# nnaisense/evotorch

Hardware: NVIDIA H100
Metric: PGPE generations/sec at popsize=1Mxdim=10k (Rastrigin, fp32) (higher is better)
Workload: dtype f32

## Files before the change

evotorch_b200/csrc/evok_common.cuh:

```cuda
#pragma once

#include <cuda_runtime.h>
#include <stdint.h>

#include "../../include/evok.h"
#include "evok_sampler.cuh"

#define EVOK_CHECK_LAUNCH_N(n)                       \
  do {                                               \
    cudaError_t e__ = cudaPeekAtLastError();         \
    if (e__ != cudaSuccess) return (int)e__;         \
    evok::count_launches(n);                         \
  } while (0)
#define EVOK_CHECK_LAUNCH() EVOK_CHECK_LAUNCH_N(1)

namespace evok {

extern unsigned long long g_launch_count;
inline void count_launches(int n) { __atomic_fetch_add(&g_launch_count, (unsigned long long)n, __ATOMIC_RELAXED); }

constexpr int kWarp = 32;
constexpr int kNumSMs = 132;
constexpr int64_t kMaxGridY = 65535;

template <typename Fn>
inline int for_item_chunks(int64_t n_items, int64_t max_items, Fn&& fn) {
  for (int64_t b0 = 0; b0 < n_items; b0 += max_items) {
    const int rc = fn(b0, n_items - b0 < max_items ? n_items - b0 : max_items);
    if (rc) return rc;
  }
  return 0;
}

inline PhiloxKey make_philox_key(uint64_t seed, uint64_t stream_id) {
  PhiloxKey k;
  uint32_t a = (uint32_t)seed, b = (uint32_t)(seed >> 32) ^ (uint32_t)(stream_id >> 32);
  for (int r = 0; r < 10; ++r) {
    k.k0[r] = a;
    k.k1[r] = b;
    a += 0x9E3779B9u;
    b += 0xBB67AE85u;
  }
  k.stream_lo = (uint32_t)stream_id;
  return k;
}

template <typename T>
__device__ __forceinline__ T block_sum(T v, T* smem ) {
  const int lane = threadIdx.x & 31, wid = threadIdx.x >> 5, nw = (blockDim.x + 31) >> 5;
  v = warp_sum(v);
  __syncthreads();
  if (lane == 0) smem[wid] = v;
  __syncthreads();
  if (wid == 0) {
    T t = lane < nw ? smem[lane] : T(0);
    t = warp_sum(t);
    if (lane == 0) smem[32] = t;
  }
  __syncthreads();
  return smem[32];
}

inline bool aligned16(const void* p) { return (reinterpret_cast<uintptr_t>(p) & 15u) == 0; }
__device__ __forceinline__ bool aligned16_dev(const void* p) { return (reinterpret_cast<uintptr_t>(p) & 15u) == 0; }

__device__ __forceinline__ float tanh_1e6(float x) {
  const float ax = fabsf(x);
  float r;
  if (ax < 0.25f) {
    const float t = ax * ax;
    r = ax * fmaf(t, fmaf(t, fmaf(t, fmaf(t, 0.021869488f, -0.053968254f), 0.13333334f), -0.33333334f), 1.0f);
  } else {
    const float e = __expf(-2.0f * ax);
    r = __fdividef(1.0f - e, 1.0f + e);
  }
  return copysignf(r, x);
}
__device__ __forceinline__ float tanh_abs1e7(float x) {
  const float e = __expf(-2.0f * fabsf(x));
  return copysignf(__fdividef(1.0f - e, 1.0f + e), x);
}
__device__ __forceinline__ float activate_fast(float v, int act) {
  switch (act) {
    case EVOK_ACT_TANH: return tanh_1e6(v);
    case EVOK_ACT_RELU: return fmaxf(v, 0.0f);
    case EVOK_ACT_SIGMOID: return __fdividef(1.0f, 1.0f + __expf(-v));
    default: return v;
  }
}

}
```

evotorch_b200/csrc/evok_grad.cu:

```cuda
#include <dlfcn.h>

#include <atomic>
#include <cstdlib>

#include "evok_common.cuh"

#ifndef EVOK_GRAD_TMA_DEFAULT
#define EVOK_GRAD_TMA_DEFAULT 1
#endif

namespace evok {

constexpr int kGradThreads = 256;
constexpr int kGradUnroll = 4;
constexpr int kGradMinBlocks = 4;
constexpr int kGradCtasPerSm = 4;
constexpr int kMaxResidentCtas = kNumSMs * 8;

template <int VEC>
struct VecF;
template <>
struct VecF<4> {
  float v[4];
};
// ... 160 lines not shown
        }
      }
    }
  }

  __shared__ float red[TY > 1 ? TY : 1][TX][2 * VEC];
  if (TY > 1) {
#pragma unroll
    for (int c = 0; c < VEC; ++c) {
      red[ty][tx][c] = s1[c];
      red[ty][tx][VEC + c] = s2[c];
    }
    __syncthreads();
    if (ty == 0) {
#pragma unroll
      for (int c = 0; c < VEC; ++c) {
        float t1 = red[0][tx][c], t2 = red[0][tx][VEC + c];
        for (int y = 1; y < TY; ++y) {
          t1 += red[y][tx][c];
          t2 += red[y][tx][VEC + c];
        }
        s1[c] = t1;
        s2[c] = t2;
      }
    }
  }
  if (ty == 0 && active) store_partial<VEC>(partial, blockIdx.y, D, col, s1, s2);
  if (SEPW && blockIdx.x == 0) {
    __shared__ float wred[TY];
    if (tx == 0) wred[ty] = wb;
    __syncthreads();
    if (threadIdx.x == 0) {
      float t = wred[0];
      for (int y = 1; y < TY; ++y) t += wred[y];
      wsum_partial[blockIdx.y] = t;
    }
  }
}

__device__ __forceinline__ void sum_chunks(const float* __restrict__ partial, int n_chunks, int64_t D, int64_t j, float& t1, float& t2) {
  t1 = 0.0f;
  t2 = 0.0f;
  for (int c = 0; c < n_chunks; ++c) {
    t1 += partial[((int64_t)c * 2 + 0) * D + j];
    t2 += partial[((int64_t)c * 2 + 1) * D + j];
  }
}

template <bool WSUM = false>
__global__ void __launch_bounds__(256) grad_finalize_kernel(const float* __restrict__ partial, int n_chunks, int64_t D, float scale_mu,
                                                            float scale_sigma, float* __restrict__ out_mu, float* __restrict__ out_sigma,
                                                            int64_t item_stride_partial = 0, const float* __restrict__ wsum_partial = nullptr,
                                                            float* __restrict__ wsum_out = nullptr) {
  const int64_t j = (int64_t)blockIdx.x * blockDim.x + threadIdx.x;
  if (WSUM && j == 0) {
    wsum_partial += (int64_t)blockIdx.y * n_chunks;
    float t = 0.0f;
    for (int c = 0; c < n_chunks; ++c) t += wsum_partial[c];
    wsum_out[blockIdx.y] = t;
  }
  if (j >= D) return;
  partial += (int64_t)blockIdx.y * item_stride_partial;
  out_mu += (int64_t)blockIdx.y * D;
  out_sigma += (int64_t)blockIdx.y * D;
  float t1, t2;
  sum_chunks(partial, n_chunks, D, j, t1, t2);
  out_mu[j] = t1 * scale_mu;
  out_sigma[j] = t2 * scale_sigma;
}

template <int EPS>
__global__ void __launch_bounds__(256) sepcma_sqnorm_kernel(const float* __restrict__ X, int64_t item_stride_x, int64_t ldx, const float* __restrict__ m,
                                                            const float* __restrict__ s, const float* __restrict__ aw, int64_t n_rows, int64_t D,
                                                            const __grid_constant__ PhiloxKey key, float* __restrict__ q) {
  const int lane = threadIdx.x & 31;
  const int64_t row = (int64_t)blockIdx.x * 8 + (threadIdx.x >> 5);
  if (row >= n_rows) return;
  const int64_t item = blockIdx.y;
  aw += item * n_rows;
  q += item * n_rows;
  if (!(__ldg(aw + row) < 0.0f)) return;
  m += item * D;
  s += item * D;
  const float* x_row = EPS == kEpsRead ? X + item * item_stride_x + row * ldx : nullptr;
  const bool vec = EPS == kEpsRead && (D & 3) == 0 && aligned16_dev(x_row);
  const uint32_t sw = key.stream_lo + (uint32_t)item;
  float acc = 0.0f;
  for (int64_t g = lane; 4 * g < D; g += 32) {
    const int64_t col = 4 * g;
    float x[4];
    if (EPS == kEpsRebuild) {
      float z[4];
      normals4(key, sw, (uint64_t)row, (uint32_t)g, z);
#pragma unroll
      for (int c = 0; c < 4; ++c) x[c] = col + c < D ? fmaf(__ldg(s + col + c), z[c], __ldg(m + col + c)) : 0.0f;
    } else if (vec) {
      const float4 v = ld_stream4(x_row + col);
      x[0] = v.x; x[1] = v.y; x[2] = v.z; x[3] = v.w;
    } else {
#pragma unroll
      for (int c = 0; c < 4; ++c) x[c] = col + c < D ? ld_stream1(x_row + col + c) : 0.0f;
    }
#pragma unroll
    for (int c = 0; c < 4; ++c) {
      if (col + c < D) {
        const float z = __fdiv_rn(x[c] - __ldg(m + col + c), __ldg(s + col + c));
        acc = fmaf(z, z, acc);
      }
    }
  }
  acc = warp_sum(acc);
  if (lane == 0) q[row] = acc;
}

struct GradPush {
  PeerSink sink;
  const unsigned long long* epoch;
  unsigned int* done;
};

__global__ void __launch_bounds__(256) grad_finalize_push_kernel(const float* __restrict__ partial, int n_chunks, int64_t D, float scale_mu,
                                                                 float scale_sigma, const __grid_constant__ PeerSink sink,
                                                                 const unsigned long long* epoch, unsigned int* done) {
  const int64_t j = (int64_t)blockIdx.x * blockDim.x + threadIdx.x;
  if (j < D) {
    float t1, t2;
    sum_chunks(partial, n_chunks, D, j, t1, t2);
    t1 *= scale_mu;
    t2 *= scale_sigma;
    for (int p = 0; p < sink.world; ++p) {
      float* slot = static_cast<float*>(sink.data[p]) + (int64_t)sink.rank * 2 * D;
      slot[j] = t1;
      slot[D + j] = t2;
    }
  }
  peer_signal_tail(sink, epoch, done);
}

#ifndef EVOK_GRAD_TMA_ROWS
#define EVOK_GRAD_TMA_ROWS 4
#endif
#ifndef EVOK_GRAD_TMA_STAGES
#define EVOK_GRAD_TMA_STAGES 4
#endif
#ifndef EVOK_GRAD_TMA_CTAS_PER_SM
#define EVOK_GRAD_TMA_CTAS_PER_SM 3
#endif
constexpr int kTmaRows = EVOK_GRAD_TMA_ROWS;
constexpr int kTmaStages = EVOK_GRAD_TMA_STAGES;
constexpr int kTmaCols = 1024;
constexpr int kTmaConsumers = 256;
constexpr int kTmaThreads = kTmaConsumers + 32;
constexpr size_t kTmaSmemBytes = (size_t)kTmaStages * kTmaRows * kTmaCols * sizeof(float) + 2 * kTmaStages * sizeof(uint64_t) + 128;

__device__ __forceinline__ uint32_t smem_u32(const void* p) { return (uint32_t)__cvta_generic_to_shared(p); }
__device__ __forceinline__ void mbar_init(uint64_t* bar, uint32_t count) {
  asm volatile("mbarrier.init.shared::cta.b64 [%0], %1;" ::"r"(smem_u32(bar)), "r"(count) : "memory");
}
__device__ __forceinline__ void mbar_expect_tx(uint64_t* bar, uint32_t bytes) {
  asm volatile("mbarrier.arrive.expect_tx.shared::cta.b64 _, [%0], %1;" ::"r"(smem_u32(bar)), "r"(bytes) : "memory");
}
__device__ __forceinline__ void mbar_arrive(uint64_t* bar) {
  asm volatile("mbarrier.arrive.shared::cta.b64 _, [%0];" ::"r"(smem_u32(bar)) : "memory");
}
__device__ __forceinline__ void mbar_wait(uint64_t* bar, uint32_t parity) {
  asm volatile(
      "{\n"
      ".reg .pred P1;\n"
      "LAB_WAIT:\n"
      "mbarrier.try_wait.parity.shared::cta.b64 P1, [%0], %1;\n"
      "@P1 bra DONE;\n"
      "bra LAB_WAIT;\n"
      "DONE:\n"
      "}" ::"r"(smem_u32(bar)), "r"(parity) : "memory");
}
__device__ __forceinline__ void bulk_load(void* dst_smem, const void* src_gmem, uint32_t bytes, uint64_t* bar) {
  asm volatile("cp.async.bulk.shared::cluster.global.mbarrier::complete_tx::bytes [%0], [%1], %2, [%3];" ::"r"(smem_u32(dst_smem)),
               "l"(src_gmem), "r"(bytes), "r"(smem_u32(bar))
               : "memory");
}

constexpr int kSplitPeriod = 16;
__device__ __forceinline__ uint32_t rebuilt_mask(int split) {
  uint32_t m = 0;
#pragma unroll
  for (int k = 0; k < kSplitPeriod; ++k)
    if ((k + 1) * split / kSplitPeriod > k * split / kSplitPeriod) m |= 1u << k;
  return m;
}
__device__ __forceinline__ bool group_rebuilt(uint32_t mask, int64_t g) { return (mask >> ((int)g & (kSplitPeriod - 1))) & 1u; }

template <bool SYM>
__global__ void __launch_bounds__(kTmaThreads, EVOK_GRAD_TMA_CTAS_PER_SM)
    grad_partial_tma_kernel(int form, const float* __restrict__ X, int64_t ldx, const float* __restrict__ w, const float* __restrict__ mu,
                            const float* __restrict__ sigma, int64_t n_units, int64_t D, int64_t units_per_chunk, int split, uint64_t unit0,
                            const __grid_constant__ PhiloxKey key, const uint32_t* __restrict__ stream_off, float* __restrict__ partial) {
  extern __shared__ __align__(128) unsigned char smem_raw[];
  float* tiles = reinterpret_cast<float*>(smem_raw);
  uint64_t* full = reinterpret_cast<uint64_t*>(smem_raw + (size_t)kTmaStages * kTmaRows * kTmaCols * sizeof(float));
  uint64_t* empty = full + kTmaStages;

  const int tid = threadIdx.x, warp = tid >> 5, lane = tid & 31;
  const int64_t col0 = (int64_t)blockIdx.x * kTmaCols;
  const int64_t width = min((int64_t)kTmaCols, D - col0);
  const int64_t r_begin = (int64_t)blockIdx.y * units_per_chunk;
  const int64_t r_end = min(n_units, r_begin + units_per_chunk);
  const int64_t n_rows = r_end - r_begin;
  const int64_t n_groups = (n_rows + kTmaRows - 1) / kTmaRows;
  const int64_t row_stride = (SYM ? 2 : 1) * ldx;
  const uint32_t mask = rebuilt_mask(split);

  if (tid == 0) {
    for (int s = 0; s < kTmaStages; ++s) {
      mbar_init(&full[s], 1);
      mbar_init(&empty[s], kTmaConsumers / 32);
    }
    asm volatile("fence.mbarrier_init.release.cluster;" ::: "memory");
  }
  __syncthreads();

  if (warp == kTmaConsumers / 32) {
    if (lane == 0) {
      const uint32_t row_bytes = (uint32_t)(width * sizeof(float));
      int64_t t = 0;
      for (int64_t g = 0; g < n_groups; ++g) {
        if (group_rebuilt(mask, g)) continue;
        const int s = (int)(t % kTmaStages);
        const uint32_t use = (uint32_t)(t / kTmaStages);
        ++t;
        if (use > 0) mbar_wait(&empty[s], (use - 1) & 1);
        const int64_t r0 = r_begin + g * kTmaRows;
        const int rows = (int)min((int64_t)kTmaRows, r_end - r0);
        mbar_expect_tx(&full[s], rows * row_bytes);
        float* dst = tiles + (size_t)s * kTmaRows * kTmaCols;
        for (int i = 0; i < rows; ++i) bulk_load(dst + (size_t)i * kTmaCols, X + (r0 + i) * row_stride + col0, row_bytes, &full[s]);
      }
    }
    return;
  }

  const int64_t col = col0 + (int64_t)tid * 4;
  const bool active = col < D;
  const uint32_t sw = key.stream_lo + (stream_off ? __ldg(stream_off) : 0u);
  const int frm = SYM ? EVOK_GRAD_SYMMETRIC : form;
  float m[4], sg[4], c1[4], c0[4];
#pragma unroll
  for (int c = 0; c < 4; ++c) {
    sg[c] = active ? __ldg(sigma + col + c) : 1.0f;
    m[c] = active ? __ldg(mu + col + c) : 0.0f;
    grad_coeffs(frm, sg[c], c1[c], c0[c]);
  }
  float s1[4] = {0.f, 0.f, 0.f, 0.f}, s2[4] = {0.f, 0.f, 0.f, 0.f};

  int64_t t = 0;
// ... 177 lines not shown
  if (chunks < p.n_chunks && !c.wsum) set_chunks(p, chunks);
  if (c.eps == kEpsRebuild && !vec_ok) {
    p.vec = 4;
    p.n_coltiles = (int)(((c.D + 3) / 4 + p.tx - 1) / p.tx);
  }
  return p;
}

using PartialKernel = void (*)(int, const float*, int64_t, const float*, const float*, const float*, int64_t, int64_t, int64_t, uint64_t,
                               PhiloxKey, const uint32_t*, float*, GradItems, SepWeights);
#define EVOK_GRAD_TXS(VEC, SYM, EPS, SEPW)                                                                             \
  {                                                                                                                    \
    grad_partial_kernel<VEC, 32, SYM, EPS, SEPW>, grad_partial_kernel<VEC, 64, SYM, EPS, SEPW>,                        \
        grad_partial_kernel<VEC, 128, SYM, EPS, SEPW>, grad_partial_kernel<VEC, 256, SYM, EPS, SEPW>                   \
  }
static const PartialKernel kPartialKernels[12][4] = {
    EVOK_GRAD_TXS(1, false, kEpsRead, false),    EVOK_GRAD_TXS(1, true, kEpsRead, false),  EVOK_GRAD_TXS(4, false, kEpsRead, false),
    EVOK_GRAD_TXS(4, true, kEpsRead, false),     EVOK_GRAD_TXS(4, false, kEpsRegen, false), EVOK_GRAD_TXS(4, true, kEpsRegen, false),
    EVOK_GRAD_TXS(4, false, kEpsRebuild, false), EVOK_GRAD_TXS(4, true, kEpsRebuild, false), EVOK_GRAD_TXS(4, false, kEpsRegen, true),
    EVOK_GRAD_TXS(1, false, kEpsRead, true),     EVOK_GRAD_TXS(4, false, kEpsRead, true),  EVOK_GRAD_TXS(4, false, kEpsRebuild, true)};
#undef EVOK_GRAD_TXS

static int partial_row(int eps, int vec, bool sym, bool sepw) {
  if (sepw) return eps == kEpsRegen ? 8 : eps == kEpsRead ? 9 + vec / 4 : 11;
  return 2 * (eps == kEpsRead ? vec / 4 : 1 + eps) + (sym ? 1 : 0);
}
static int tx_index(int tx) { return tx == 32 ? 0 : tx == 64 ? 1 : tx == 128 ? 2 : 3; }

static void launch_partial(const GradCall& c, const GradPlan& p, int64_t b0, int64_t nb, float* partial) {
  PhiloxKey key = c.key;
  key.stream_lo += (uint32_t)b0;
  const float* X = c.X + b0 * c.items.x;
  const float* w = c.w + b0 * c.items.w;
  const float* mu = c.mu + b0 * c.items.mu;
  const float* sigma = c.sigma + b0 * c.items.sigma;
  const uint64_t unit0 = (uint64_t)(is_sym(c) ? c.row0 / 2 : c.row0);
  if (p.tma) {
    const int rebuilt = c.split < 0 ? device_auto_split() : c.split;
    auto kernel = is_sym(c) ? grad_partial_tma_kernel<true> : grad_partial_tma_kernel<false>;
    cudaFuncSetAttribute(kernel, cudaFuncAttributeMaxDynamicSharedMemorySize, (int)kTmaSmemBytes);
    kernel<<<dim3(p.n_coltiles, p.n_chunks), kTmaThreads, kTmaSmemBytes, c.st>>>(c.form, X, c.ldx, w, mu, sigma, p.n_units, c.D, p.units_per_chunk,
                                                                                  rebuilt, unit0, key, c.stream_off, partial);
    return;
  }
  SepWeights sepw = c.sepw;
  if (sepw.q) sepw.q += b0 * c.items.w;
  const PartialKernel kernel = kPartialKernels[partial_row(c.eps, p.vec, is_sym(c), c.wsum != nullptr)][tx_index(p.tx)];
  kernel<<<dim3(p.n_coltiles, p.n_chunks, (unsigned)nb), kGradThreads, 0, c.st>>>(c.form, X, c.ldx, w, mu, sigma, p.n_units, c.D,
                                                                                    p.units_per_chunk, unit0, key, c.stream_off, partial, c.items, sepw);
}

static int launch_finalize(const GradCall& c, int n_chunks, int64_t b0, int64_t nb, const float* partial) {
  const unsigned grid = (unsigned)((c.D + 255) / 256);
  if (c.push) {
    grad_finalize_push_kernel<<<grid, 256, 0, c.st>>>(partial, n_chunks, c.D, c.scale_mu, c.scale_sigma, c.push->sink, c.push->epoch, c.push->done);
  } else if (c.wsum) {
    grad_finalize_kernel<true><<<dim3(grid, (unsigned)nb), 256, 0, c.st>>>(partial, n_chunks, c.D, c.scale_mu, c.scale_sigma, c.out_mu + b0 * c.D,
                                                                           c.out_sigma + b0 * c.D, c.items.partial, c.sepw.wsum_partial, c.wsum + b0);
  } else {
    grad_finalize_kernel<<<dim3(grid, (unsigned)nb), 256, 0, c.st>>>(partial, n_chunks, c.D, c.scale_mu, c.scale_sigma, c.out_mu + b0 * c.D,
                                                                     c.out_sigma + b0 * c.D, c.items.partial);
  }
  EVOK_CHECK_LAUNCH();
  return 0;
}

static int run_grad(GradCall c) {
  if (c.n_items == 0) return 0;
  float* partial = (float*)c.ws;
  if ((is_sym(c) ? c.n_rows / 2 : c.n_rows) == 0) {
    if (c.push) return launch_finalize(c, 0, 0, 1, partial);
    cudaMemsetAsync(c.out_mu, 0, (size_t)c.n_items * c.D * 4, c.st);
    cudaMemsetAsync(c.out_sigma, 0, (size_t)c.n_items * c.D * 4, c.st);
    return 0;
  }
  const GradPlan p = plan_grad(c);
  c.items.partial = (int64_t)p.n_chunks * 2 * c.D;
  const int64_t chunk = c.n_items < kMaxGridY ? c.n_items : kMaxGridY;
  if (c.ws_bytes < (size_t)chunk * c.items.partial * sizeof(float)) return EVOK_E_WORKSPACE;
  return for_item_chunks(c.n_items, kMaxGridY, [&](int64_t b0, int64_t nb) {
    launch_partial(c, p, b0, nb, partial);
    EVOK_CHECK_LAUNCH();
    return launch_finalize(c, p.n_chunks, b0, nb, partial);
  });
}

static bool bad_form(int form) { return form < EVOK_GRAD_SEPARABLE || form > EVOK_GRAD_MOMENTS; }

static int grad_single(const GradCall& c) {
  const bool read = c.eps == kEpsRead;
  if ((!c.w && c.n_rows != 0) || !c.mu || !c.sigma || !c.ws || (read && !c.X) || (!c.push && (!c.out_mu || !c.out_sigma))) return EVOK_E_NULLPTR;
  if (bad_form(c.form)) return EVOK_E_BADENUM;
  if (c.n_rows < 0 || c.D <= 0 || c.row0 < 0 || (read && c.ldx < c.D) || c.split < -1 || c.split > kSplitPeriod) return EVOK_E_BADSIZE;
  if (is_sym(c) && ((c.n_rows & 1) || (c.row0 & 1))) return EVOK_E_ODDROWS;
  if (c.ws_bytes < evok_grad_workspace_bytes(c.n_rows, c.D)) return EVOK_E_WORKSPACE;
  return run_grad(c);
}

static int grad_batched(const GradCall& c) {
  const bool read = c.eps == kEpsRead;
  if ((read && !c.X) || !c.w || !c.mu || !c.sigma || !c.out_mu || !c.out_sigma || !c.ws) return EVOK_E_NULLPTR;
  if (bad_form(c.form)) return EVOK_E_BADENUM;
  if (c.n_items < 0 || c.n_rows < 0 || c.D <= 0 || (read && c.ldx < c.D) || c.items.x < 0 || c.items.mu < 0 || c.items.sigma < 0)
    return EVOK_E_BADSIZE;
  if (is_sym(c) && (c.n_rows & 1)) return EVOK_E_ODDROWS;
  return run_grad(c);
}

}

using namespace evok;

extern "C" EVOK_API size_t evok_grad_workspace_bytes(int64_t n_rows, int64_t D) {
  (void)n_rows;
  if (D <= 0) return 256;
// ... 182 lines not shown
```

evotorch_b200/csrc/evok_rank.cu:

```cuda
#include "evok_common.cuh"

namespace evok {

constexpr int kRadixBits = 8;
constexpr int kRadix = 1 << kRadixBits;
constexpr int kSortThreads = 256;
constexpr int kSortWarps = kSortThreads / 32;
constexpr int kItemsPerThread = 8;
constexpr int kTile = kSortThreads * kItemsPerThread;

__device__ __forceinline__ uint32_t orderable(float v) {
  if (v != v) return 0xFFFFFFFFu;
  v += 0.0f;
  const uint32_t b = __float_as_uint(v);
  return (b & 0x80000000u) ? ~b : (b | 0x80000000u);
}

__device__ __forceinline__ uint32_t sort_key(float f, int descending) {
  const uint32_t k = orderable(f);
  return descending ? ~k : k;
}

__global__ void __launch_bounds__(256) make_keys_kernel(const float* __restrict__ f, int64_t N, int descending,
                                                        uint32_t* __restrict__ keys, uint32_t* __restrict__ idx) {
  const int64_t i = (int64_t)blockIdx.x * blockDim.x + threadIdx.x;
  if (i < N) {
    keys[i] = sort_key(f[i], descending);
    idx[i] = (uint32_t)i;
  }
}

__global__ void __launch_bounds__(kSortThreads) radix_hist_kernel(const uint32_t* __restrict__ keys, int64_t N, int shift,
                                                                  uint32_t* __restrict__ counts, int n_tiles) {
  __shared__ uint32_t h[kRadix];
  for (int i = threadIdx.x; i < kRadix; i += kSortThreads) h[i] = 0;
  __syncthreads();
  const int64_t base = (int64_t)blockIdx.x * kTile;
#pragma unroll
  for (int it = 0; it < kItemsPerThread; ++it) {
    const int64_t i = base + it * kSortThreads + threadIdx.x;
    if (i < N) atomicAdd(&h[(keys[i] >> shift) & (kRadix - 1)], 1u);
  }
  __syncthreads();
  for (int d = threadIdx.x; d < kRadix; d += kSortThreads) counts[(int64_t)d * n_tiles + blockIdx.x] = h[d];
}

constexpr int kSelfScanMaxTiles = 256;

template <bool FIRST>
__global__ void __launch_bounds__(kSortThreads)
    radix_hist_t_kernel(const float* __restrict__ f, int descending, uint32_t* __restrict__ keys, uint32_t* __restrict__ idx, int64_t N, int shift,
                        uint32_t* __restrict__ counts_t) {
  __shared__ uint32_t h[kRadix];
  for (int i = threadIdx.x; i < kRadix; i += kSortThreads) h[i] = 0;
  __syncthreads();
  const int64_t base = (int64_t)blockIdx.x * kTile;
#pragma unroll
  for (int it = 0; it < kItemsPerThread; ++it) {
    const int64_t i = base + it * kSortThreads + threadIdx.x;
    if (i < N) {
      uint32_t k;
      if (FIRST) {
        k = sort_key(f[i], descending);
        keys[i] = k;
        idx[i] = (uint32_t)i;
      } else {
        k = keys[i];
      }
      atomicAdd(&h[(k >> shift) & (kRadix - 1)], 1u);
    }
  }
  __syncthreads();
  for (int d = threadIdx.x; d < kRadix; d += kSortThreads) counts_t[(int64_t)blockIdx.x * kRadix + d] = h[d];
}

__global__ void __launch_bounds__(256) digit_scan_kernel(uint32_t* __restrict__ counts, int n_tiles, uint32_t* __restrict__ totals) {
  __shared__ uint32_t warp_tot[8];
  __shared__ uint32_t carry_s, chunk_s;
  uint32_t* row = counts + (int64_t)blockIdx.x * n_tiles;
  const int lane = threadIdx.x & 31, wid = threadIdx.x >> 5;
  if (threadIdx.x == 0) carry_s = 0;
  __syncthreads();
  for (int base = 0; base < n_tiles; base += 256) {
    const int i = base + threadIdx.x;
    const uint32_t v = i < n_tiles ? row[i] : 0u;
    uint32_t incl = v;
#pragma unroll
    for (int o = 1; o < 32; o <<= 1) {
      const uint32_t t = __shfl_up_sync(0xffffffffu, incl, o);
      if (lane >= o) incl += t;
    }
    if (lane == 31) warp_tot[wid] = incl;
    __syncthreads();
    if (wid == 0) {
      const uint32_t t = lane < 8 ? warp_tot[lane] : 0u;
      uint32_t ti = t;
#pragma unroll
      for (int o = 1; o < 8; o <<= 1) {
        const uint32_t u = __shfl_up_sync(0xffffffffu, ti, o);
        if (lane >= o) ti += u;
      }
      if (lane < 8) warp_tot[lane] = ti - t;
      if (lane == 7) chunk_s = ti;
    }
    __syncthreads();
    const uint32_t carry = carry_s;
    if (i < n_tiles) row[i] = carry + warp_tot[wid] + incl - v;
    __syncthreads();
    if (threadIdx.x == 0) carry_s = carry + chunk_s;
    __syncthreads();
  }
  if (threadIdx.x == 0) totals[blockIdx.x] = carry_s;
}

template <bool SELF_SCAN>
__global__ void __launch_bounds__(kSortThreads)
    radix_scatter_kernel(const uint32_t* __restrict__ keys_in, const uint32_t* __restrict__ idx_in, uint32_t* __restrict__ keys_out,
                         uint32_t* __restrict__ idx_out, int64_t N, int shift, const uint32_t* __restrict__ offsets, int n_tiles,
                         const uint32_t* __restrict__ totals) {
  __shared__ uint32_t wcount[kSortWarps][kRadix];
  __shared__ uint32_t digit_base[kRadix];
  __shared__ uint32_t wtot[kSortWarps];
  __shared__ uint32_t tile_prefix[kRadix];
  const int lane = threadIdx.x & 31, wid = threadIdx.x >> 5;
  for (int i = threadIdx.x; i < kSortWarps * kRadix; i += kSortThreads) (&wcount[0][0])[i] = 0;
  {
    uint32_t t;
    if (SELF_SCAN) {
      uint32_t before = 0, all = 0;
      for (int tile = 0; tile < n_tiles; ++tile) {
        const uint32_t c = offsets[(int64_t)tile * kRadix + threadIdx.x];
        all += c;
        before += tile < (int)blockIdx.x ? c : 0u;
      }
      tile_prefix[threadIdx.x] = before;
      t = all;
    } else {
      t = totals[threadIdx.x];
    }
    uint32_t incl = t;
#pragma unroll
    for (int o = 1; o < 32; o <<= 1) {
      const uint32_t u = __shfl_up_sync(0xffffffffu, incl, o);
      if (lane >= o) incl += u;
    }
    if (lane == 31) wtot[wid] = incl;
    __syncthreads();
    uint32_t wb = 0;
#pragma unroll
    for (int w = 0; w < kSortWarps; ++w) wb += w < wid ? wtot[w] : 0u;
    digit_base[threadIdx.x] = wb + incl - t;
  }
  __syncthreads();

  const int64_t wbase = (int64_t)blockIdx.x * kTile + (int64_t)wid * (32 * kItemsPerThread);
  uint32_t key[kItemsPerThread], val[kItemsPerThread], rnk[kItemsPerThread];
#pragma unroll
  for (int it = 0; it < kItemsPerThread; ++it) {
    const int64_t i = wbase + it * 32 + lane;
    const bool ok = i < N;
    key[it] = ok ? keys_in[i] : 0xFFFFFFFFu;
    val[it] = ok ? idx_in[i] : 0u;
    const uint32_t d = (key[it] >> shift) & (kRadix - 1);
    const uint32_t peers = __match_any_sync(0xffffffffu, ok ? d : (kRadix + 1u));
    const uint32_t below = __popc(peers & ((1u << lane) - 1u));
    uint32_t base = 0;
    if (ok && below == 0) {
      base = wcount[wid][d];
      wcount[wid][d] = base + __popc(peers);
    }
    base = __shfl_sync(0xffffffffu, base, __ffs(peers) - 1);
    rnk[it] = base + below;
    __syncwarp();
  }
  __syncthreads();
  for (int d = threadIdx.x; d < kRadix; d += kSortThreads) {
    uint32_t run = digit_base[d] + (SELF_SCAN ? tile_prefix[d] : offsets[(int64_t)d * n_tiles + blockIdx.x]);
#pragma unroll
    for (int w = 0; w < kSortWarps; ++w) {
      const uint32_t c = wcount[w][d];
      wcount[w][d] = run;
      run += c;
    }
  }
  __syncthreads();
#pragma unroll
  for (int it = 0; it < kItemsPerThread; ++it) {
    const int64_t i = wbase + it * 32 + lane;
    if (i < N) {
      const uint32_t d = (key[it] >> shift) & (kRadix - 1);
      const uint32_t pos = wcount[wid][d] + rnk[it];
      keys_out[pos] = key[it];
      idx_out[pos] = val[it];
    }
  }
}

__device__ __forceinline__ float nes_term(int64_t p, float Nf, float top) { return fmaxf(0.0f, top - logf(Nf - (float)p)); }

__device__ __forceinline__ double nes_partial_sum(int64_t N, int64_t first, int stride) {
  const float Nf = (float)N, top = logf(Nf / 2.0f + 1.0f);
  double acc = 0.0;
  for (int64_t p = first; p < N; p += stride) acc += (double)nes_term(p, Nf, top);
  return acc;
}

__device__ __forceinline__ float utility_at(int64_t p, int64_t N, int method, const float* nes_sum) {
  if (method == EVOK_RANK_CENTERED) return __fdiv_rn((float)p, (float)(N - 1)) - 0.5f;
  if (method == EVOK_RANK_LINEAR) return __fdiv_rn((float)p, (float)(N - 1));
  const float Nf = (float)N;
  return __fdiv_rn(nes_term(p, Nf, logf(Nf / 2.0f + 1.0f)), *nes_sum) - __fdiv_rn(1.0f, Nf);
}

enum { kUtilities = 0, kArgsort = 1, kEliteMask = 2, kTable = 3 };

struct Emit {
  int mode;
  int method;
  int64_t num_elites;
  float* out;
  int64_t* perm;
  const float* table;
  __host__ __device__ Emit item(int64_t off) const {
    Emit e = *this;
    if (out) e.out += off;
    if (perm) e.perm += off;
    return e;
  }
};

static Emit utilities(int method, float* w, int64_t* perm) { return Emit{kUtilities, method, 0, w, perm, nullptr}; }
static Emit permutation(int64_t* perm) { return Emit{kArgsort, 0, 0, nullptr, perm, nullptr}; }
static Emit elite_flags(int64_t num_elites, float* mask) { return Emit{kEliteMask, 0, num_elites, mask, nullptr, nullptr}; }
static Emit table_entries(const float* table, float* out) { return Emit{kTable, 0, 0, out, nullptr, table}; }

__device__ __forceinline__ void emit_at(int64_t p, uint32_t i, int64_t N, const Emit& e, const float* nes_sum) {
  if (e.perm) e.perm[p] = (int64_t)i;
  if (e.mode == kUtilities) e.out[i] = utility_at(p, N, e.method, nes_sum);
  else if (e.mode == kEliteMask) e.out[i] = p < e.num_elites ? 1.0f : 0.0f;
  else if (e.mode == kTable) e.out[i] = e.table[p];
}

__global__ void __launch_bounds__(1024) nes_table_sum_kernel(int64_t N, float* __restrict__ out_sum) {
  __shared__ double sm[33];
  const double tot = block_sum<double>(nes_partial_sum(N, threadIdx.x, 1024), sm);
  if (threadIdx.x == 0) *out_sum = (float)tot;
}

__global__ void __launch_bounds__(256) scatter_sorted_kernel(const uint32_t* __restrict__ idx, int64_t N, const Emit e,
                                                             const float* __restrict__ nes_sum) {
  const int64_t p = (int64_t)blockIdx.x * blockDim.x + threadIdx.x;
  if (p < N) emit_at(p, idx[p], N, e, nes_sum);
}

__global__ void __launch_bounds__(1024) mean_std_kernel(const float* __restrict__ f, int64_t N, float sign, float* __restrict__ stats) {
  __shared__ double sm[33];
  f += (int64_t)blockIdx.x * N;
  stats += 2 * blockIdx.x;
  double s = 0.0;
  for (int64_t i = threadIdx.x; i < N; i += 1024) s += (double)(sign * f[i]);
  const double mean = block_sum<double>(s, sm) / (double)N;
  double q = 0.0;
  for (int64_t i = threadIdx.x; i < N; i += 1024) {
    const double d = (double)(sign * f[i]) - mean;
    q += d * d;
  }
  const double var = block_sum<double>(q, sm) / (double)(N - 1);
  if (threadIdx.x == 0) {
    stats[0] = (float)mean;
    stats[1] = (float)sqrt(var);
  }
}
__global__ void __launch_bounds__(256) affine_kernel(const float* __restrict__ f, int64_t N, float sign, const float* __restrict__ stats,
                                                     int normalized, float* __restrict__ w) {
  const int64_t i = (int64_t)blockIdx.x * blockDim.x + threadIdx.x;
  if (i >= N) return;
  f += (int64_t)blockIdx.y * N;
  w += (int64_t)blockIdx.y * N;
  stats += 2 * blockIdx.y;
  const float g = sign * f[i];
  w[i] = normalized ? __fdiv_rn(g - stats[0], stats[1]) : g;
}

__global__ void __launch_bounds__(1024) weights_adjust_kernel(float* __restrict__ w, int64_t N, int mode) {
  __shared__ double sm[33];
  w += (int64_t)blockIdx.x * N;
  double s = 0.0;
  for (int64_t i = threadIdx.x; i < N; i += 1024) s += mode == 1 ? (double)w[i] : (double)fabsf(w[i]);
  const double tot = block_sum<double>(s, sm);
  if (mode == 1) {
    const float mean = (float)(tot / (double)N);
    for (int64_t i = threadIdx.x; i < N; i += 1024) w[i] -= mean;
  } else {
    const float d = (float)tot;
    for (int64_t i = threadIdx.x; i < N; i += 1024) w[i] = __fdiv_rn(w[i], d);
  }
}

constexpr int kSmallRankMax = 8192;
constexpr int kSmallThreads = 256;
constexpr int kSmallTile = 2048;

template <int PARTS>
// ... 28 lines not shown
  if (e.mode == kUtilities && e.method == EVOK_RANK_NES)
    nes_sum = (float)block_sum<double>(nes_partial_sum(N, threadIdx.x, kSmallThreads), red);
  if (i < N && part == 0) emit_at(cnt, (uint32_t)i, N, e, &nes_sum);
}

static int rank_small(const float* f, int64_t N, int64_t n_items, int descending, const Emit& e, cudaStream_t st) {
  if (N <= 1024) {
    rank_small_kernel<4><<<dim3((unsigned)((N + 63) / 64), (unsigned)n_items), kSmallThreads, 0, st>>>(f, (int)N, descending, e);
  } else if (N <= 4096) {
    rank_small_kernel<8><<<dim3((unsigned)((N + 31) / 32), (unsigned)n_items), kSmallThreads, 0, st>>>(f, (int)N, descending, e);
  } else {
    rank_small_kernel<16><<<dim3((unsigned)((N + 15) / 16), (unsigned)n_items), kSmallThreads, 0, st>>>(f, (int)N, descending, e);
  }
  EVOK_CHECK_LAUNCH();
  return 0;
}

struct SortPlan {
  int64_t N;
  int n_tiles;
  size_t off_keys0, off_keys1, off_idx0, off_idx1, off_counts, off_totals, off_scalar, total;
};

static SortPlan make_plan(int64_t N) {
  SortPlan p;
  p.N = N;
  p.n_tiles = (int)((N + kTile - 1) / kTile);
  if (p.n_tiles < 1) p.n_tiles = 1;
  auto al = [](size_t x) { return (x + 255) & ~(size_t)255; };
  size_t o = 0;
  p.off_keys0 = o; o += al((size_t)N * 4);
  p.off_keys1 = o; o += al((size_t)N * 4);
  p.off_idx0 = o; o += al((size_t)N * 4);
  p.off_idx1 = o; o += al((size_t)N * 4);
  p.off_counts = o; o += al((size_t)kRadix * p.n_tiles * 4);
  p.off_totals = o; o += al((size_t)kRadix * 4);
  p.off_scalar = o; o += 64 + 2 * kNumSMs * 8 + 192;
  p.total = o;
  return p;
}

static int sort_pairs(const float* f, int64_t N, int descending, void* ws, const SortPlan& p, cudaStream_t st, uint32_t** sorted_idx,
                      uint32_t** sorted_keys = nullptr) {
  char* base = (char*)ws;
  uint32_t* keys[2] = {(uint32_t*)(base + p.off_keys0), (uint32_t*)(base + p.off_keys1)};
  uint32_t* idx[2] = {(uint32_t*)(base + p.off_idx0), (uint32_t*)(base + p.off_idx1)};
  uint32_t* counts = (uint32_t*)(base + p.off_counts);
  uint32_t* totals = (uint32_t*)(base + p.off_totals);
  const bool self_scan = p.n_tiles <= kSelfScanMaxTiles;
  if (!self_scan) {
    make_keys_kernel<<<(unsigned)((N + 255) / 256), 256, 0, st>>>(f, N, descending, keys[0], idx[0]);
    EVOK_CHECK_LAUNCH();
  }
  int cur = 0;
  for (int pass = 0; pass < 32 / kRadixBits; ++pass) {
    const int shift = pass * kRadixBits;
    if (self_scan) {
      if (pass == 0) radix_hist_t_kernel<true><<<p.n_tiles, kSortThreads, 0, st>>>(f, descending, keys[0], idx[0], N, shift, counts);
      else radix_hist_t_kernel<false><<<p.n_tiles, kSortThreads, 0, st>>>(nullptr, 0, keys[cur], nullptr, N, shift, counts);
      radix_scatter_kernel<true><<<p.n_tiles, kSortThreads, 0, st>>>(keys[cur], idx[cur], keys[cur ^ 1], idx[cur ^ 1], N, shift, counts, p.n_tiles, totals);
      EVOK_CHECK_LAUNCH_N(2);
    } else {
      radix_hist_kernel<<<p.n_tiles, kSortThreads, 0, st>>>(keys[cur], N, shift, counts, p.n_tiles);
      digit_scan_kernel<<<kRadix, 256, 0, st>>>(counts, p.n_tiles, totals);
      radix_scatter_kernel<false><<<p.n_tiles, kSortThreads, 0, st>>>(keys[cur], idx[cur], keys[cur ^ 1], idx[cur ^ 1], N, shift, counts, p.n_tiles, totals);
      EVOK_CHECK_LAUNCH_N(3);
    }
    cur ^= 1;
  }
  *sorted_idx = idx[cur];
  if (sorted_keys) *sorted_keys = keys[cur];
  return 0;
}

static int rank_rows(const float* keys, int64_t N, int64_t n_items, int descending, const Emit& e, void* ws, size_t ws_bytes,
                     cudaStream_t st) {
  if (N <= kSmallRankMax)
    return for_item_chunks(n_items, kMaxGridY, [&](int64_t b0, int64_t nb) {
      return rank_small(keys + b0 * N, N, nb, descending, e.item(b0 * N), st);
    });
  const SortPlan p = make_plan(N);
  if (ws_bytes < p.total) return EVOK_E_WORKSPACE;
  float* nes_sum = (float*)((char*)ws + p.off_scalar);
  const bool nes = e.mode == kUtilities && e.method == EVOK_RANK_NES;
  for (int64_t b = 0; b < n_items; ++b) {
    uint32_t* sidx = nullptr;
    const int rc = sort_pairs(keys + b * N, N, descending, ws, p, st, &sidx);
    if (rc) return rc;
    if (nes) nes_table_sum_kernel<<<1, 1024, 0, st>>>(N, nes_sum);
    scatter_sorted_kernel<<<(unsigned)((N + 255) / 256), 256, 0, st>>>(sidx, N, e.item(b * N), nes_sum);
    EVOK_CHECK_LAUNCH_N(nes ? 2 : 1);
  }
  return 0;
}

static int affine_rows(int method, const float* f, int64_t N, int64_t n_items, int higher_is_better, float* w, float* stats, cudaStream_t st) {
  const float sign = higher_is_better ? 1.0f : -1.0f;
  const int normalized = method == EVOK_RANK_NORMALIZED;
  return for_item_chunks(n_items, kMaxGridY, [&](int64_t b0, int64_t nb) {
    const float* fc = f + b0 * N;
    if (normalized) mean_std_kernel<<<(unsigned)nb, 1024, 0, st>>>(fc, N, sign, stats);
    affine_kernel<<<dim3((unsigned)((N + 255) / 256), (unsigned)nb), 256, 0, st>>>(fc, N, sign, stats, normalized, w + b0 * N);
    EVOK_CHECK_LAUNCH_N(normalized ? 2 : 1);
    return 0;
  });
}

struct ShardTable {
  long long off[EVOK_MAX_PEERS + 1];
};

constexpr int kRankPushThreads = 1024;

__global__ void __launch_bounds__(kRankPushThreads)
    rank_push_kernel(const uint32_t* __restrict__ sorted_keys, const float* __restrict__ f, int64_t n_local, int64_t my_off,
                     const __grid_constant__ PeerSink keys_sink, const __grid_constant__ PeerSink fsum_sink, const unsigned long long* epoch) {
  __shared__ double red[33];
  const int p = (keys_sink.rank + 1 + blockIdx.x) % keys_sink.world;
  uint32_t* dst = static_cast<uint32_t*>(keys_sink.data[p]) + my_off;
  if (((reinterpret_cast<uintptr_t>(dst) | reinterpret_cast<uintptr_t>(sorted_keys)) & 15u) == 0) {
    const int64_t nq = n_local >> 2;
    for (int64_t q = threadIdx.x; q < nq; q += kRankPushThreads) reinterpret_cast<uint4*>(dst)[q] = reinterpret_cast<const uint4*>(sorted_keys)[q];
    for (int64_t i = (nq << 2) + threadIdx.x; i < n_local; i += kRankPushThreads) dst[i] = sorted_keys[i];
  } else {
    for (int64_t i = threadIdx.x; i < n_local; i += kRankPushThreads) dst[i] = sorted_keys[i];
  }
  double acc = 0.0;
  for (int64_t i = threadIdx.x; i < n_local; i += kRankPushThreads) acc += (double)f[i];
  const double tot = block_sum<double>(acc, red);
  if (threadIdx.x == 0) {
    static_cast<double*>(fsum_sink.data[p])[keys_sink.rank] = tot;
    __threadfence_system();
    st_release_sys(keys_sink.flags[p] + keys_sink.rank, *epoch + 1ull);
  }
}

__device__ __forceinline__ unsigned long long rank_timer_ns() {
  unsigned long long t;
  asm volatile("mov.u64 %0, %globaltimer;" : "=l"(t));
  return t;
}

__global__ void __launch_bounds__(256)
// ... 210 lines not shown
```

Measured before the change: 55.63.

## Use programmatic dependent launch across sort and gradient kernels; stage radix scatter in smem

Launches the radix sort passes, rank scatter and gradient finalize kernels with programmatic stream serialization, adding griddepcontrol wait/launch_dependents so each kernel's launch and prologue can overlap the tail of the previous one. The radix scatter kernel is restructured to stage keys and values in shared memory in digit order and then write them out contiguously, for more coalesced global stores. The histogram kernel now loads keys before its atomics. This adds shared memory use in scatter and depends on correct placement of the PDL wait calls.

Result: no change. 55.83, median of 6 (+0.4%).

```diff
diff --git a/evotorch_b200/csrc/evok_common.cuh b/evotorch_b200/csrc/evok_common.cuh
--- a/evotorch_b200/csrc/evok_common.cuh
+++ b/evotorch_b200/csrc/evok_common.cuh
@@ -2,6 +2,8 @@
 
 #include <cuda_runtime.h>
 #include <stdint.h>
+
+#include <utility>
 
 #include "../../include/evok.h"
 #include "evok_sampler.cuh"
@@ -61,6 +63,24 @@
   return smem[32];
 }
 
+__device__ __forceinline__ void pdl_wait() { asm volatile("griddepcontrol.wait;" ::: "memory"); }
+__device__ __forceinline__ void pdl_launch_dependents() { asm volatile("griddepcontrol.launch_dependents;" ::: "memory"); }
+
+template <typename... Params, typename... Args>
+inline cudaError_t launch_dependent(void (*kernel)(Params...), dim3 grid, dim3 block, size_t smem, cudaStream_t st, Args&&... args) {
+  cudaLaunchAttribute attr[1];
+  attr[0].id = cudaLaunchAttributeProgrammaticStreamSerialization;
+  attr[0].val.programmaticStreamSerializationAllowed = 1;
+  cudaLaunchConfig_t cfg = {};
+  cfg.gridDim = grid;
+  cfg.blockDim = block;
+  cfg.dynamicSmemBytes = smem;
+  cfg.stream = st;
+  cfg.attrs = attr;
+  cfg.numAttrs = 1;
+  return cudaLaunchKernelEx(&cfg, kernel, std::forward<Args>(args)...);
+}
+
 inline bool aligned16(const void* p) { return (reinterpret_cast<uintptr_t>(p) & 15u) == 0; }
 __device__ __forceinline__ bool aligned16_dev(const void* p) { return (reinterpret_cast<uintptr_t>(p) & 15u) == 0; }
 
diff --git a/evotorch_b200/csrc/evok_grad.cu b/evotorch_b200/csrc/evok_grad.cu
--- a/evotorch_b200/csrc/evok_grad.cu
+++ b/evotorch_b200/csrc/evok_grad.cu
@@ -236,6 +236,7 @@
                                                             float scale_sigma, float* __restrict__ out_mu, float* __restrict__ out_sigma,
                                                             int64_t item_stride_partial = 0, const float* __restrict__ wsum_partial = nullptr,
                                                             float* __restrict__ wsum_out = nullptr) {
+  pdl_wait();
   const int64_t j = (int64_t)blockIdx.x * blockDim.x + threadIdx.x;
   if (WSUM && j == 0) {
     wsum_partial += (int64_t)blockIdx.y * n_chunks;
@@ -306,6 +307,7 @@
 __global__ void __launch_bounds__(256) grad_finalize_push_kernel(const float* __restrict__ partial, int n_chunks, int64_t D, float scale_mu,
                                                                  float scale_sigma, const __grid_constant__ PeerSink sink,
                                                                  const unsigned long long* epoch, unsigned int* done) {
+  pdl_wait();
   const int64_t j = (int64_t)blockIdx.x * blockDim.x + threadIdx.x;
   if (j < D) {
     float t1, t2;
@@ -384,6 +386,7 @@
   uint64_t* full = reinterpret_cast<uint64_t*>(smem_raw + (size_t)kTmaStages * kTmaRows * kTmaCols * sizeof(float));
   uint64_t* empty = full + kTmaStages;
 
+  pdl_launch_dependents();
   const int tid = threadIdx.x, warp = tid >> 5, lane = tid & 31;
   const int64_t col0 = (int64_t)blockIdx.x * kTmaCols;
   const int64_t width = min((int64_t)kTmaCols, D - col0);
@@ -667,15 +670,18 @@
 
 static int launch_finalize(const GradCall& c, int n_chunks, int64_t b0, int64_t nb, const float* partial) {
   const unsigned grid = (unsigned)((c.D + 255) / 256);
+  cudaError_t e;
   if (c.push) {
-    grad_finalize_push_kernel<<<grid, 256, 0, c.st>>>(partial, n_chunks, c.D, c.scale_mu, c.scale_sigma, c.push->sink, c.push->epoch, c.push->done);
+    e = launch_dependent(grad_finalize_push_kernel, dim3(grid), dim3(256), 0, c.st, partial, n_chunks, c.D, c.scale_mu, c.scale_sigma, c.push->sink,
+                         c.push->epoch, c.push->done);
   } else if (c.wsum) {
-    grad_finalize_kernel<true><<<dim3(grid, (unsigned)nb), 256, 0, c.st>>>(partial, n_chunks, c.D, c.scale_mu, c.scale_sigma, c.out_mu + b0 * c.D,
-                                                                           c.out_sigma + b0 * c.D, c.items.partial, c.sepw.wsum_partial, c.wsum + b0);
+    e = launch_dependent(grad_finalize_kernel<true>, dim3(grid, (unsigned)nb), dim3(256), 0, c.st, partial, n_chunks, c.D, c.scale_mu, c.scale_sigma,
+                         c.out_mu + b0 * c.D, c.out_sigma + b0 * c.D, c.items.partial, c.sepw.wsum_partial, c.wsum + b0);
   } else {
-    grad_finalize_kernel<<<dim3(grid, (unsigned)nb), 256, 0, c.st>>>(partial, n_chunks, c.D, c.scale_mu, c.scale_sigma, c.out_mu + b0 * c.D,
-                                                                     c.out_sigma + b0 * c.D, c.items.partial);
-  }
+    e = launch_dependent(grad_finalize_kernel<false>, dim3(grid, (unsigned)nb), dim3(256), 0, c.st, partial, n_chunks, c.D, c.scale_mu, c.scale_sigma,
+                         c.out_mu + b0 * c.D, c.out_sigma + b0 * c.D, c.items.partial, nullptr, nullptr);
+  }
+  if (e != cudaSuccess) return (int)e;
   EVOK_CHECK_LAUNCH();
   return 0;
 }
diff --git a/evotorch_b200/csrc/evok_rank.cu b/evotorch_b200/csrc/evok_rank.cu
--- a/evotorch_b200/csrc/evok_rank.cu
+++ b/evotorch_b200/csrc/evok_rank.cu
@@ -23,6 +23,7 @@
 
 __global__ void __launch_bounds__(256) make_keys_kernel(const float* __restrict__ f, int64_t N, int descending,
                                                         uint32_t* __restrict__ keys, uint32_t* __restrict__ idx) {
+  pdl_launch_dependents();
   const int64_t i = (int64_t)blockIdx.x * blockDim.x + threadIdx.x;
   if (i < N) {
     keys[i] = sort_key(f[i], descending);
@@ -33,14 +34,20 @@
 __global__ void __launch_bounds__(kSortThreads) radix_hist_kernel(const uint32_t* __restrict__ keys, int64_t N, int shift,
                                                                   uint32_t* __restrict__ counts, int n_tiles) {
   __shared__ uint32_t h[kRadix];
+  pdl_wait();
+  pdl_launch_dependents();
   for (int i = threadIdx.x; i < kRadix; i += kSortThreads) h[i] = 0;
   __syncthreads();
   const int64_t base = (int64_t)blockIdx.x * kTile;
+  uint32_t k[kItemsPerThread];
 #pragma unroll
   for (int it = 0; it < kItemsPerThread; ++it) {
     const int64_t i = base + it * kSortThreads + threadIdx.x;
-    if (i < N) atomicAdd(&h[(keys[i] >> shift) & (kRadix - 1)], 1u);
-  }
+    k[it] = i < N ? keys[i] : 0u;
+  }
+#pragma unroll
+  for (int it = 0; it < kItemsPerThread; ++it)
+    if (base + it * kSortThreads + threadIdx.x < N) atomicAdd(&h[(k[it] >> shift) & (kRadix - 1)], 1u);
   __syncthreads();
   for (int d = threadIdx.x; d < kRadix; d += kSortThreads) counts[(int64_t)d * n_tiles + blockIdx.x] = h[d];
 }
@@ -52,6 +59,8 @@
     radix_hist_t_kernel(const float* __restrict__ f, int descending, uint32_t* __restrict__ keys, uint32_t* __restrict__ idx, int64_t N, int shift,
                         uint32_t* __restrict__ counts_t) {
   __shared__ uint32_t h[kRadix];
+  pdl_wait();
+  pdl_launch_dependents();
   for (int i = threadIdx.x; i < kRadix; i += kSortThreads) h[i] = 0;
   __syncthreads();
   const int64_t base = (int64_t)blockIdx.x * kTile;
@@ -77,6 +86,8 @@
 __global__ void __launch_bounds__(256) digit_scan_kernel(uint32_t* __restrict__ counts, int n_tiles, uint32_t* __restrict__ totals) {
   __shared__ uint32_t warp_tot[8];
   __shared__ uint32_t carry_s, chunk_s;
+  pdl_wait();
+  pdl_launch_dependents();
   uint32_t* row = counts + (int64_t)blockIdx.x * n_tiles;
   const int lane = threadIdx.x & 31, wid = threadIdx.x >> 5;
   if (threadIdx.x == 0) carry_s = 0;
@@ -113,54 +124,70 @@
   if (threadIdx.x == 0) totals[blockIdx.x] = carry_s;
 }
 
+__device__ __forceinline__ uint32_t cta_exclusive_scan(uint32_t t, uint32_t* wtot) {
+  const int lane = threadIdx.x & 31, wid = threadIdx.x >> 5;
+  uint32_t incl = t;
+#pragma unroll
+  for (int o = 1; o < 32; o <<= 1) {
+    const uint32_t u = __shfl_up_sync(0xffffffffu, incl, o);
+    if (lane >= o) incl += u;
+  }
+  if (lane == 31) wtot[wid] = incl;
+  __syncthreads();
+  uint32_t wb = 0;
+#pragma unroll
+  for (int w = 0; w < kSortWarps; ++w) wb += w < wid ? wtot[w] : 0u;
+  __syncthreads();
+  return wb + incl - t;
+}
+
 template <bool SELF_SCAN>
 __global__ void __launch_bounds__(kSortThreads)
     radix_scatter_kernel(const uint32_t* __restrict__ keys_in, const uint32_t* __restrict__ idx_in, uint32_t* __restrict__ keys_out,
                          uint32_t* __restrict__ idx_out, int64_t N, int shift, const uint32_t* __restrict__ offsets, int n_tiles,
                          const uint32_t* __restrict__ totals) {
+  static_assert(kSortThreads == kRadix, "thread d owns digit d");
   __shared__ uint32_t wcount[kSortWarps][kRadix];
-  __shared__ uint32_t digit_base[kRadix];
   __shared__ uint32_t wtot[kSortWarps];
-  __shared__ uint32_t tile_prefix[kRadix];
-  const int lane = threadIdx.x & 31, wid = threadIdx.x >> 5;
+  __shared__ uint32_t tile_base[kRadix];
+  __shared__ uint32_t out_shift[kRadix];
+  __shared__ uint32_t staged_key[kTile], staged_val[kTile];
+  pdl_wait();
+  pdl_launch_dependents();
+  const int lane = threadIdx.x & 31, wid = threadIdx.x >> 5, d_own = threadIdx.x;
   for (int i = threadIdx.x; i < kSortWarps * kRadix; i += kSortThreads) (&wcount[0][0])[i] = 0;
+  uint32_t out_base;
   {
     uint32_t t;
     if (SELF_SCAN) {
       uint32_t before = 0, all = 0;
       for (int tile = 0; tile < n_tiles; ++tile) {
-        const uint32_t c = offsets[(int64_t)tile * kRadix + threadIdx.x];
+        const uint32_t c = offsets[(int64_t)tile * kRadix + d_own];
         all += c;
         before += tile < (int)blockIdx.x ? c : 0u;
       }
-      tile_prefix[threadIdx.x] = before;
+      out_base = before;
       t = all;
     } else {
-      t = totals[threadIdx.x];
-    }
-    uint32_t incl = t;
-#pragma unroll
-    for (int o = 1; o < 32; o <<= 1) {
-      const uint32_t u = __shfl_up_sync(0xffffffffu, incl, o);
-      if (lane >= o) incl += u;
-    }
-    if (lane == 31) wtot[wid] = incl;
-    __syncthreads();
-    uint32_t wb = 0;
-#pragma unroll
-    for (int w = 0; w < kSortWarps; ++w) wb += w < wid ? wtot[w] : 0u;
-    digit_base[threadIdx.x] = wb + incl - t;
-  }
-  __syncthreads();
-
-  const int64_t wbase = (int64_t)blockIdx.x * kTile + (int64_t)wid * (32 * kItemsPerThread);
+      t = totals[d_own];
+      out_base = offsets[(int64_t)d_own * n_tiles + blockIdx.x];
+    }
+    out_base += cta_exclusive_scan(t, wtot);
+  }
+
+  const int64_t tile0 = (int64_t)blockIdx.x * kTile;
+  const int wbase = wid * (32 * kItemsPerThread);
+  const int valid = (int)min((int64_t)kTile, N - tile0);
   uint32_t key[kItemsPerThread], val[kItemsPerThread], rnk[kItemsPerThread];
 #pragma unroll
   for (int it = 0; it < kItemsPerThread; ++it) {
-    const int64_t i = wbase + it * 32 + lane;
-    const bool ok = i < N;
-    key[it] = ok ? keys_in[i] : 0xFFFFFFFFu;
-    val[it] = ok ? idx_in[i] : 0u;
+    const int t = wbase + it * 32 + lane;
+    key[it] = t < valid ? keys_in[tile0 + t] : 0xFFFFFFFFu;
+    val[it] = t < valid ? idx_in[tile0 + t] : 0u;
+  }
+#pragma unroll
+  for (int it = 0; it < kItemsPerThread; ++it) {
+    const bool ok = wbase + it * 32 + lane < valid;
     const uint32_t d = (key[it] >> shift) & (kRadix - 1);
     const uint32_t peers = __match_any_sync(0xffffffffu, ok ? d : (kRadix + 1u));
     const uint32_t below = __popc(peers & ((1u << lane) - 1u));
@@ -174,25 +201,34 @@
     __syncwarp();
   }
   __syncthreads();
-  for (int d = threadIdx.x; d < kRadix; d += kSortThreads) {
-    uint32_t run = digit_base[d] + (SELF_SCAN ? tile_prefix[d] : offsets[(int64_t)d * n_tiles + blockIdx.x]);
+  {
+    uint32_t run = 0;
 #pragma unroll
     for (int w = 0; w < kSortWarps; ++w) {
-      const uint32_t c = wcount[w][d];
-      wcount[w][d] = run;
+      const uint32_t c = wcount[w][d_own];
+      wcount[w][d_own] = run;
       run += c;
     }
+    const uint32_t first = cta_exclusive_scan(run, wtot);
+    tile_base[d_own] = first;
+    out_shift[d_own] = out_base - first;
   }
   __syncthreads();
 #pragma unroll
   for (int it = 0; it < kItemsPerThread; ++it) {
-    const int64_t i = wbase + it * 32 + lane;
-    if (i < N) {
+    if (wbase + it * 32 + lane < valid) {
       const uint32_t d = (key[it] >> shift) & (kRadix - 1);
-      const uint32_t pos = wcount[wid][d] + rnk[it];
-      keys_out[pos] = key[it];
-      idx_out[pos] = val[it];
-    }
+      const uint32_t slot = tile_base[d] + wcount[wid][d] + rnk[it];
+      staged_key[slot] = key[it];
+      staged_val[slot] = val[it];
+    }
+  }
+  __syncthreads();
+  for (int slot = threadIdx.x; slot < valid; slot += kSortThreads) {
+    const uint32_t k = staged_key[slot];
+    const uint32_t pos = out_shift[(k >> shift) & (kRadix - 1)] + (uint32_t)slot;
+    keys_out[pos] = k;
+    idx_out[pos] = staged_val[slot];
   }
 }
 
@@ -243,12 +279,16 @@
 
 __global__ void __launch_bounds__(1024) nes_table_sum_kernel(int64_t N, float* __restrict__ out_sum) {
   __shared__ double sm[33];
+  pdl_wait();
+  pdl_launch_dependents();
   const double tot = block_sum<double>(nes_partial_sum(N, threadIdx.x, 1024), sm);
   if (threadIdx.x == 0) *out_sum = (float)tot;
 }
 
 __global__ void __launch_bounds__(256) scatter_sorted_kernel(const uint32_t* __restrict__ idx, int64_t N, const Emit e,
                                                              const float* __restrict__ nes_sum) {
+  pdl_wait();
+  pdl_launch_dependents();
   const int64_t p = (int64_t)blockIdx.x * blockDim.x + threadIdx.x;
   if (p < N) emit_at(p, idx[p], N, e, nes_sum);
 }
@@ -383,18 +423,26 @@
     make_keys_kernel<<<(unsigned)((N + 255) / 256), 256, 0, st>>>(f, N, descending, keys[0], idx[0]);
     EVOK_CHECK_LAUNCH();
   }
+  const dim3 tiles(p.n_tiles), threads(kSortThreads);
   int cur = 0;
   for (int pass = 0; pass < 32 / kRadixBits; ++pass) {
     const int shift = pass * kRadixBits;
+    cudaError_t e = cudaSuccess;
     if (self_scan) {
-      if (pass == 0) radix_hist_t_kernel<true><<<p.n_tiles, kSortThreads, 0, st>>>(f, descending, keys[0], idx[0], N, shift, counts);
-      else radix_hist_t_kernel<false><<<p.n_tiles, kSortThreads, 0, st>>>(nullptr, 0, keys[cur], nullptr, N, shift, counts);
-      radix_scatter_kernel<true><<<p.n_tiles, kSortThreads, 0, st>>>(keys[cur], idx[cur], keys[cur ^ 1], idx[cur ^ 1], N, shift, counts, p.n_tiles, totals);
+      if (pass == 0) radix_hist_t_kernel<true><<<tiles, threads, 0, st>>>(f, descending, keys[0], idx[0], N, shift, counts);
+      else e = launch_dependent(radix_hist_t_kernel<false>, tiles, threads, 0, st, nullptr, 0, keys[cur], nullptr, N, shift, counts);
+      if (e == cudaSuccess)
+        e = launch_dependent(radix_scatter_kernel<true>, tiles, threads, 0, st, keys[cur], idx[cur], keys[cur ^ 1], idx[cur ^ 1], N, shift, counts,
+                             p.n_tiles, totals);
+      if (e != cudaSuccess) return (int)e;
       EVOK_CHECK_LAUNCH_N(2);
     } else {
-      radix_hist_kernel<<<p.n_tiles, kSortThreads, 0, st>>>(keys[cur], N, shift, counts, p.n_tiles);
-      digit_scan_kernel<<<kRadix, 256, 0, st>>>(counts, p.n_tiles, totals);
-      radix_scatter_kernel<false><<<p.n_tiles, kSortThreads, 0, st>>>(keys[cur], idx[cur], keys[cur ^ 1], idx[cur ^ 1], N, shift, counts, p.n_tiles, totals);
+      e = launch_dependent(radix_hist_kernel, tiles, threads, 0, st, keys[cur], N, shift, counts, p.n_tiles);
+      if (e == cudaSuccess) e = launch_dependent(digit_scan_kernel, dim3(kRadix), dim3(256), 0, st, counts, p.n_tiles, totals);
+      if (e == cudaSuccess)
+        e = launch_dependent(radix_scatter_kernel<false>, tiles, threads, 0, st, keys[cur], idx[cur], keys[cur ^ 1], idx[cur ^ 1], N, shift, counts,
+                             p.n_tiles, totals);
+      if (e != cudaSuccess) return (int)e;
       EVOK_CHECK_LAUNCH_N(3);
     }
     cur ^= 1;
@@ -418,8 +466,9 @@
     uint32_t* sidx = nullptr;
     const int rc = sort_pairs(keys + b * N, N, descending, ws, p, st, &sidx);
     if (rc) return rc;
-    if (nes) nes_table_sum_kernel<<<1, 1024, 0, st>>>(N, nes_sum);
-    scatter_sorted_kernel<<<(unsigned)((N + 255) / 256), 256, 0, st>>>(sidx, N, e.item(b * N), nes_sum);
+    cudaError_t err = nes ? launch_dependent(nes_table_sum_kernel, dim3(1), dim3(1024), 0, st, N, nes_sum) : cudaSuccess;
+    if (err == cudaSuccess) err = launch_dependent(scatter_sorted_kernel, dim3((unsigned)((N + 255) / 256)), dim3(256), 0, st, sidx, N, e.item(b * N), nes_sum);
+    if (err != cudaSuccess) return (int)err;
     EVOK_CHECK_LAUNCH_N(nes ? 2 : 1);
   }
   return 0;
```
